# georgeretsi/smirk

Hardware: AMD Instinct MI355X
Metric: faces/sec (encode+FLAME+render+generate) @224x224 (higher is better)
Workload: dtype f32 results; encoder + generator convs as split-fp16 x3 MFMA with f32 accumulate (fp32-class error), FLAME / raster f32; 1 GPU; BASELINE config 4: full inference incl. SmirkGenerator re-synthesis, 1024-frame batch sharded over the GPUs; global_batch=1024, micro_batch=1024, image=224x224, parallelism=dp1, rccl_ranks_seen=1, collective=none (1 GPU), hw_queues=4

## Files before the change

### smirk_amd/csrc/mbconv_image.hip

```cpp
#include <stdio.h>

#include "common.h"

typedef _Float16 half8 __attribute__((ext_vector_type(8)));

struct MBIArgs {
    const char* x;
    const char* wexp;
    const float *s1, *b1;
    const float* wdw;
    const float *s2, *b2;
    const char* wproj;
    const float *s3, *b3;
    char* out;
    int B, H, W, Cin, mid, Cout, residual, ipw, rows, gsz, nb;
    int off_es, off_wp, off_wc, off_gmap;
    int gpitch;
    int tile, tiles_x, tiles_y, nbands;
};

extern __shared__ __attribute__((aligned(16))) char mbi_smem[];

__device__ __forceinline__ void mbi_barrier() {
    asm volatile("s_waitcnt lgkmcnt(0)" ::: "memory");
    __builtin_amdgcn_s_barrier();
    asm volatile("" ::: "memory");
}

__device__ __forceinline__ int mbi_es(int gi, int c) { return gi * 32 + ((((c >> 2) ^ (gi >> 1)) & 7) << 2) + (c & 3); }

template <int KS, int NT, bool PADK>
__device__ __forceinline__ void mbi_whole_body(const MBIArgs& a) {
    SmirkRangeAccS rng;
    const int strideX = KS * 64 + 16;
    char* Xs = mbi_smem;
    float* Es = (float*)(mbi_smem + a.off_es);
    char* Wp = mbi_smem + a.off_wp;
    float* Wc = (float*)(mbi_smem + a.off_wc);
    short* gmap = (short*)(mbi_smem + a.off_gmap);
    const int tid = threadIdx.x, lane = tid & 63, wave = tid >> 6, fr = lane & 31, hb = lane >> 5;
    const int b0 = blockIdx.x * a.ipw;
    const int nimg = min(a.ipw, a.B - b0), HW = a.H * a.W, vrows = nimg * HW;
    const int nchunks = (a.mid + 31) / 32;
    const size_t xrow = (size_t)a.Cin * 4;
    const half8 hz = {0, 0, 0, 0, 0, 0, 0, 0};
    const int swave = __builtin_amdgcn_readfirstlane(wave);
    const bool active = swave < a.nb;
    const int wpbuf = a.Cout * 144;

    half8 we[KS][2];
    float s1v = 0.f, b1v = 0.f;
    auto load_we = [&](int c) {
        int frw = fr;
        asm volatile("" : "+v"(frw));
        const int ch = 32 * c + frw;
        const bool v = ch < a.mid;
        const int chc = min(ch, a.mid - 1);
        const char* wbase = a.wexp;
        asm volatile("" : "+s"(wbase));
        const char* wrow = wbase + (unsigned)chc * (unsigned)(a.Cin * 4);
#pragma unroll
        for (int s = 0; s < KS; ++s) {
            const int g = 2 * s + hb;
            if constexpr (PADK) {
                const int gc = min(g, a.Cin / 8 - 1);
                const half8 t0 = *(const half8*)(wrow + gc * 32), t1h = *(const half8*)(wrow + gc * 32 + 16);
                we[s][0] = g * 8 < a.Cin ? t0 : hz;
                we[s][1] = g * 8 < a.Cin ? t1h : hz;
            } else {
                we[s][0] = *(const half8*)(wrow + g * 32);
                we[s][1] = *(const half8*)(wrow + g * 32 + 16);
            }
        }
        const float t1 = a.s1[chc], t2 = a.b1[chc];
        s1v = v ? t1 : 0.f;
        b1v = v ? t2 : 0.f;
    };
    f32x4 wpv[2];
    float wcv = 0.f;
    auto fetch_stage = [&](int c) {
        int t0 = tid;
        asm volatile("" : "+v"(t0));
#pragma unroll
        for (int u = 0; u < 2; ++u) {
            const int idx = t0 + 512 * u, row = idx >> 3, piece = idx & 7, kg = 4 * c + (piece >> 1);
            const bool ok = row < a.Cout && kg * 8 < a.mid;
            const int rc = min(row, a.Cout - 1), kc = min(kg, a.mid / 8 - 1);
            const f32x4 t = *(const f32x4*)(a.wproj + ((size_t)rc * a.mid + kc * 8) * 4 + (piece & 1) * 16);
            const f32x4 z = {0.f, 0.f, 0.f, 0.f};
            wpv[u] = ok ? t : z;
        }
        {
            const int k = min(t0 >> 5, 10), ch = 32 * c + (t0 & 31), chc = min(ch, a.mid - 1);
            const float* src = k < 9 ? a.wdw + (size_t)k * a.mid : (k == 9 ? a.s2 : a.b2);
            const float t = src[chc];
            wcv = ch < a.mid ? t : 0.f;
        }
    };
    auto store_stage = [&](int c) {
        char* dst = Wp + (c & 1) * wpbuf;
        int t0 = tid;
        asm volatile("" : "+v"(t0));
#pragma unroll
        for (int u = 0; u < 2; ++u) {
            const int idx = t0 + 512 * u, row = idx >> 3, piece = idx & 7;
            if (row < a.Cout) *(f32x4*)(dst + row * 144 + piece * 16) = wpv[u];
        }
        if (t0 < 352) Wc[(c & 1) * 352 + t0] = wcv;
    };

    {
        const int P = a.Cin / 4;
        const char* xb = a.x + (size_t)b0 * HW * xrow;
        const int total = a.rows * P, vtotal = vrows * P;
        for (int base = 0; base < total; base += 512 * 4) {
            f32x4 xv[4];
#pragma unroll
            for (int u = 0; u < 4; ++u) {
                const int idx = base + 512 * u + tid;
                const f32x4 z = {0.f, 0.f, 0.f, 0.f};
                const f32x4 t = *(const f32x4*)(xb + (size_t)min(idx, vtotal - 1) * 16);
                xv[u] = idx < vtotal ? t : z;
            }
#pragma unroll
            for (int u = 0; u < 4; ++u) {
                const int idx = base + 512 * u + tid, row = idx / P, pc = idx - row * P;
                if (idx < total) *(f32x4*)(Xs + row * strideX + pc * 16) = xv[u];
            }
        }
        if (PADK && KS * 4 > P) {
            const int PP = KS * 4 - P;
            for (int idx = tid; idx < a.rows * PP; idx += 512) {
                const int row = idx / PP, pc = P + idx - row * PP;
                *(f32x4*)(Xs + row * strideX + pc * 16) = f32x4{0.f, 0.f, 0.f, 0.f};
            }
        }
        for (int idx = tid; idx < a.gsz * 8; idx += 512) ((f32x4*)Es)[idx] = f32x4{0.f, 0.f, 0.f, 0.f};
        for (int r = tid; r < a.nb * 32; r += 512) {
            int g = -1;
            if (r < vrows) {
                const int im = r / HW, rem = r - im * HW, y = rem / a.W, xx = rem - y * a.W;
                g = (im * (a.H + 2) + y + 1) * (a.W + 2) + xx + 1;
            }
            gmap[r] = (short)g;
        }
    }
    mbi_barrier();

    f32x16 pacc[NT][2];
#pragma unroll
    for (int q = 0; q < NT; ++q)
#pragma unroll
        for (int h = 0; h < 2; ++h)
#pragma unroll
            for (int r = 0; r < 16; ++r) pacc[q][h][r] = 0.f;
    const int myrow = min(wave * 32 + fr, a.rows - 1);
    const int mygi = active ? (int)gmap[min(wave * 32 + fr, a.nb * 32 - 1)] : -1;

    auto expand = [&]() {
        if (!active) return;
        f32x16 e0, e1;
#pragma unroll
        for (int r = 0; r < 16; ++r) { e0[r] = 0.f; e1[r] = 0.f; }
        const char* arow = Xs + myrow * strideX;
#pragma unroll
        for (int s = 0; s < KS; ++s) {
            const int g = 2 * s + hb;
            const half8 ah = *(const half8*)(arow + g * 32), al = *(const half8*)(arow + g * 32 + 16);
            e0 = __builtin_amdgcn_mfma_f32_32x32x16_f16(ah, we[s][0], e0, 0, 0, 0);
            e1 = __builtin_amdgcn_mfma_f32_32x32x16_f16(ah, we[s][1], e1, 0, 0, 0);
            e1 = __builtin_amdgcn_mfma_f32_32x32x16_f16(al, we[s][0], e1, 0, 0, 0);
            if ((s & 1) || NT == 4) __builtin_amdgcn_sched_barrier(0);
        }
        int rbase = wave * 32 + 4 * hb;
        asm volatile("" : "+v"(rbase));
#pragma unroll
        for (int r = 0; r < 16; ++r) {
            const int gm = gmap[rbase + (r & 3) + 8 * (r >> 2)];
            const float v = fmaxf((e0[r] + e1[r] * (1.0f / 2048.0f)) * s1v + b1v, 0.f);
            Es[mbi_es(gm >= 0 ? gm : ~gm, fr)] = gm >= 0 ? v : 0.f;
        }
    };


    for (int c = -1; c < nchunks; ++c) {
        const bool more = c + 1 < nchunks;
        if (more) fetch_stage(c + 1);
        half8 dh[2] = {hz, hz}, dl[2] = {hz, hz};
        if (c >= 0 && active && mygi >= 0) {
            const float* wc = Wc + (c & 1) * 352;
#pragma unroll
            for (int s = 0; s < 2; ++s) {
                const int c8 = 8 * (2 * s + hb);
                int gc = mygi;
                asm volatile("" : "+v"(gc));
                float acc[8] = {0.f, 0.f, 0.f, 0.f, 0.f, 0.f, 0.f, 0.f};
#pragma unroll
                for (int ky = 0; ky < 3; ++ky)
#pragma unroll
                    for (int kx = 0; kx < 3; ++kx) {
                        const int gi = gc + (ky - 1) * a.gpitch + (kx - 1);
                        const f32x4 v0 = *(const f32x4*)(Es + mbi_es(gi, c8)), v1 = *(const f32x4*)(Es + mbi_es(gi, c8 + 4));
                        const f32x4 w0 = *(const f32x4*)(wc + (ky * 3 + kx) * 32 + c8), w1 = *(const f32x4*)(wc + (ky * 3 + kx) * 32 + c8 + 4);
#pragma unroll
                        for (int q = 0; q < 4; ++q) { acc[q] = fmaf(v0[q], w0[q], acc[q]); acc[4 + q] = fmaf(v1[q], w1[q], acc[4 + q]); }
                        if (kx == 2 || NT == 4) __builtin_amdgcn_sched_barrier(0);
                    }
                const f32x4 sa = *(const f32x4*)(wc + 9 * 32 + c8), sb = *(const f32x4*)(wc + 9 * 32 + c8 + 4);
                const f32x4 ba = *(const f32x4*)(wc + 10 * 32 + c8), bb = *(const f32x4*)(wc + 10 * 32 + c8 + 4);
#pragma unroll
                for (int q = 0; q < 8; ++q) {
                    const float v = fmaxf(acc[q] * (q < 4 ? sa[q & 3] : sb[q & 3]) + (q < 4 ? ba[q & 3] : bb[q & 3]), 0.f);
                    _Float16 h, l;
                    smirk_split1(v, h, l);
                    dh[s][q] = h; dl[s][q] = l;
                }
            }
        }
        if (more) store_stage(c + 1);
        mbi_barrier();
        if (more) load_we(c + 1);
        if (c >= 0 && active) {
            const char* wp = Wp + (c & 1) * wpbuf;
            int frq = fr;
            asm volatile("" : "+v"(frq));
#pragma unroll
            for (int q = 0; q < NT; ++q) {
                const int co = min(q * 32 + frq, a.Cout - 1);
                const char* brow = wp + co * 144;
#pragma unroll
                for (int s = 0; s < 2; ++s) {
                    const int g = 2 * s + hb;
                    const half8 bhh = *(const half8*)(brow + g * 32), bll = *(const half8*)(brow + g * 32 + 16);
                    pacc[q][0] = __builtin_amdgcn_mfma_f32_32x32x16_f16(dh[s], bhh, pacc[q][0], 0, 0, 0);
                    pacc[q][1] = __builtin_amdgcn_mfma_f32_32x32x16_f16(dh[s], bll, pacc[q][1], 0, 0, 0);
                    pacc[q][1] = __builtin_amdgcn_mfma_f32_32x32x16_f16(dl[s], bhh, pacc[q][1], 0, 0, 0);
                }
                __builtin_amdgcn_sched_barrier(0);
            }
        }
        if (more) expand();
        mbi_barrier();
    }

    if (active) {
        const int lane = __builtin_amdgcn_mbcnt_hi(~0u, __builtin_amdgcn_mbcnt_lo(~0u, 0u)), wave = swave, fr = lane & 31;
        float* tb = Es + wave * (32 * 36);
        char* ob = a.out + (size_t)b0 * HW * a.Cout * 4;
#pragma unroll
        for (int q = 0; q < NT; ++q) {
            if (q * 32 < a.Cout) {
                const int co = q * 32 + fr;
                const float s3 = co < a.Cout ? a.s3[co] : 0.f, b3 = co < a.Cout ? a.b3[co] : 0.f;
#pragma unroll
                for (int r = 0; r < 16; ++r) tb[mfma32_row(r, lane) * 36 + fr] = (pacc[q][0][r] + pacc[q][1][r] * (1.0f / 2048.0f)) * s3 + b3;
                asm volatile("s_waitcnt lgkmcnt(0)" ::: "memory");
#pragma unroll
                for (int it = 0; it < 2; ++it) {
                    const int item = it * 64 + lane, row = item >> 2, g8 = q * 4 + (item & 3);
                    const int r = wave * 32 + row;
                    if (r < vrows && g8 * 8 < a.Cout) {
                        float v[8];
                        *(f32x4*)v = *(const f32x4*)(tb + row * 36 + (item & 3) * 8);
                        *(f32x4*)(v + 4) = *(const f32x4*)(tb + row * 36 + (item & 3) * 8 + 4);
                        if (a.residual) {
                            const char* xr = Xs + r * strideX + g8 * 32;
                            const half8 hi = *(const half8*)xr, lo = *(const half8*)(xr + 16);
#pragma unroll
                            for (int k = 0; k < 8; ++k) v[k] += (float)hi[k] + (float)lo[k] * (1.0f / 2048.0f);
                        }
                        half8 hi, lo;
                        rng.see8(v);
#pragma unroll
                        for (int k = 0; k < 8; ++k) {
                            _Float16 h, l;
                            smirk_split1(v[k], h, l);
                            hi[k] = h; lo[k] = l;
                        }
                        char* o = ob + ((size_t)r * a.Cout + g8 * 8) * 4;
                        *(half8*)o = hi;
                        *(half8*)(o + 16) = lo;
                    }
                }
                asm volatile("s_waitcnt lgkmcnt(0)" ::: "memory");
            }
        }
    }
    rng.commit();
}

#define MBB_EB 8192
#define MBB_STAGE 34

__device__ __forceinline__ void mbb_out_px(int m, int& oy, int& ox) {
    const int k = m >> 2;
    oy = (0x96 >> k) & 1;
    ox = (k >> 1) * 4 + (m & 3);
}

__device__ __forceinline__ void mbb_fence() { asm volatile("s_waitcnt lgkmcnt(0)" ::: "memory"); }

template <int KS, int NT>
__device__ __forceinline__ void mbi_band_body(const MBIArgs& a) {
    SmirkRangeAccS rng;
    const int tid = threadIdx.x, lane = tid & 63, fr = lane & 31, hb = lane >> 5;
    const int wave = __builtin_amdgcn_readfirstlane(tid >> 6);
    float* Wt = (float*)(mbi_smem + 4 * MBB_EB);
    const int band = (int)blockIdx.x * 4 + wave;
    const bool has = band < a.nbands;
    int bid = min(band, a.nbands - 1);
    const int bx = bid % a.tiles_x; bid /= a.tiles_x;
    const int by = bid % a.tiles_y;
    const int b = bid / a.tiles_y;
    const int oy0 = by * 2, ox0 = bx * 14;
    const bool interior = oy0 > 0 && oy0 + 2 < a.H && ox0 > 0 && ox0 + 14 < a.W;
    const unsigned xrow = (unsigned)a.Cin * 4;
    const int gmax = a.Cin / 8;
    const int nchunks = (a.mid + 31) / 32;
    const half8 hz = {0, 0, 0, 0, 0, 0, 0, 0};
    const char* xb = a.x + (size_t)b * a.H * a.W * xrow;

    auto stage = [&](int c0) {
        const int total = min(MBB_STAGE, nchunks - c0) * 352;
        for (int base = 0; base < total; base += 256 * 8) {
            float cv[8];
#pragma unroll
            for (int u = 0; u < 8; ++u) {
                const int idx = min(base + 256 * u + tid, total - 1), cl = idx / 352, rem = idx - cl * 352, k = rem >> 5;
                const int ch = 32 * (c0 + cl) + (rem & 31), chc = min(ch, a.mid - 1);
                const float* src = k < 9 ? a.wdw + (size_t)k * a.mid : (k == 9 ? a.s2 : a.b2);
                const float t = src[chc];
                cv[u] = ch < a.mid ? t : 0.f;
            }
#pragma unroll
            for (int u = 0; u < 8; ++u)
                if (base + 256 * u + tid < total) Wt[base + 256 * u + tid] = cv[u];
        }
    };
    unsigned xo[2], om[2];
#pragma unroll
    for (int t = 0; t < 2; ++t) {
        const int iy = oy0 - 1 + 2 * t + (fr >> 4), ix = ox0 - 1 + (fr & 15);
        const bool ok = iy >= 0 && iy < a.H && ix >= 0 && ix < a.W;
        const int yc = min(max(iy, 0), a.H - 1), xc = min(max(ix, 0), a.W - 1);
        xo[t] = (unsigned)(yc * a.W + xc) * xrow;
        om[t] = (unsigned)__builtin_amdgcn_ballot_w64(ok) >> (4 * hb);
    }
    auto load_x = [&](int t, half8 (*dst)[2]) {
        const char* px = xb + xo[t];
#pragma unroll
        for (int s = 0; s < KS; ++s) {
            const int g = 2 * s + hb, gc = min(g, gmax - 1);
            const half8 t0 = *(const half8*)(px + gc * 32), t1 = *(const half8*)(px + gc * 32 + 16);
            if (s == KS - 1) { dst[s][0] = g < gmax ? t0 : hz; dst[s][1] = g < gmax ? t1 : hz; }
            else { dst[s][0] = t0; dst[s][1] = t1; }
        }
    };
    half8 xa[2][KS][2];
    load_x(0, xa[0]);
    load_x(1, xa[1]);
    half8 we[KS][2];
    float s1v, b1v;
    auto load_we = [&](int c) {
        const int ch = 32 * c + fr, chc = min(ch, a.mid - 1);
        const char* wrow = a.wexp + (size_t)chc * xrow;
#pragma unroll
        for (int s = 0; s < KS; ++s) {
            const int g = 2 * s + hb, gc = min(g, gmax - 1);
            const half8 t0 = *(const half8*)(wrow + gc * 32), t1 = *(const half8*)(wrow + gc * 32 + 16);
            if (s == KS - 1) { we[s][0] = g < gmax ? t0 : hz; we[s][1] = g < gmax ? t1 : hz; }
            else { we[s][0] = t0; we[s][1] = t1; }
        }
        const float t1 = a.s1[chc], t2 = a.b1[chc];
        s1v = ch < a.mid ? t1 : 0.f;
        b1v = ch < a.mid ? t2 : 0.f;
    };
    load_we(0);
    stage(0);
    mbb_fence();
    __builtin_amdgcn_s_barrier();
    asm volatile("" ::: "memory");
    if (!has) {
        for (int c0 = MBB_STAGE; c0 < nchunks; c0 += MBB_STAGE) {
            __builtin_amdgcn_s_barrier();
            stage(c0);
            mbb_fence();
            __builtin_amdgcn_s_barrier();
        }
        return;
    }

    const unsigned ebase = (unsigned)wave * MBB_EB;
    const unsigned est = ebase + hb * 512 + ((((unsigned)fr >> 2) ^ (hb << 1)) << 4) + (fr & 3) * 4;
    unsigned ta[9];
    int my_oy, my_ox;
    mbb_out_px(fr, my_oy, my_ox);
#pragma unroll
    for (int ky = 0; ky < 3; ++ky)
#pragma unroll
        for (int kx = 0; kx < 3; ++kx) {
            const int cell = ((my_oy + ky) * 16 + my_ox + kx) & 63;
            ta[ky * 3 + kx] = ebase + cell * 128 + ((((cell >> 1) ^ (2 * hb)) & 7) << 4);
        }

    f32x16 pacc[NT][2];
#pragma unroll
    for (int q = 0; q < NT; ++q)
#pragma unroll
        for (int h = 0; h < 2; ++h)
#pragma unroll
            for (int r = 0; r < 16; ++r) pacc[q][h][r] = 0.f;

    const float* wc = Wt;
    int crestage = MBB_STAGE;
    for (int c = 0; c < nchunks; ++c, wc += 352) {
        if (c == crestage) {
            mbb_fence();
            __builtin_amdgcn_s_barrier();
            stage(c);
            mbb_fence();
            __builtin_amdgcn_s_barrier();
            asm volatile("" ::: "memory");
            wc = Wt; crestage += MBB_STAGE;
        }
#pragma unroll
        for (int t = 0; t < 2; ++t) {
            half8 (*cur)[2] = xa[t];
            unsigned et = est;
            asm volatile("" : "+v"(et));
            f32x16 e0, e1;
#pragma unroll
            for (int r = 0; r < 16; ++r) { e0[r] = 0.f; e1[r] = 0.f; }
#pragma unroll
            for (int s = 0; s < KS; ++s) {
                e0 = __builtin_amdgcn_mfma_f32_32x32x16_f16(cur[s][0], we[s][0], e0, 0, 0, 0);
                e1 = __builtin_amdgcn_mfma_f32_32x32x16_f16(cur[s][0], we[s][1], e1, 0, 0, 0);
                e1 = __builtin_amdgcn_mfma_f32_32x32x16_f16(cur[s][1], we[s][0], e1, 0, 0, 0);
            }
            if (interior) {
#pragma unroll
                for (int r = 0; r < 16; ++r) {
                    const int ro = (r & 3) + 8 * (r >> 2);
                    const unsigned cr = ((r >> 1) & 1) | (((r >> 2) & 1) << 2);
                    const float v = fmaxf((e0[r] + e1[r] * (1.0f / 2048.0f)) * s1v + b1v, 0.f);
                    *(float*)(mbi_smem + (et ^ (cr << 4)) + (32 * t + ro) * 128) = v;
                }
            } else {
#pragma unroll
                for (int r = 0; r < 16; ++r) {
                    const int ro = (r & 3) + 8 * (r >> 2);
                    const unsigned cr = ((r >> 1) & 1) | (((r >> 2) & 1) << 2);
                    const float v = fmaxf((e0[r] + e1[r] * (1.0f / 2048.0f)) * s1v + b1v, 0.f);
                    *(float*)(mbi_smem + (et ^ (cr << 4)) + (32 * t + ro) * 128) = ((om[t] >> ro) & 1u) ? v : 0.f;
                }
            }
        }
        if (c + 1 < nchunks) load_we(c + 1);
        half8 wp[NT][2][2];
#pragma unroll
        for (int q = 0; q < NT; ++q) {
            const int co = q * 32 + fr;
            const char* wrow = a.wproj + (size_t)(co < a.Cout ? co : 0) * a.mid * 4;
#pragma unroll
            for (int s = 0; s < 2; ++s) {
                const int kg = min(4 * c + 2 * s + hb, a.mid / 8 - 1);
                const bool v = co < a.Cout && (4 * c + 2 * s + hb) * 8 < a.mid;
                const half8 t0 = *(const half8*)(wrow + kg * 32), t1 = *(const half8*)(wrow + kg * 32 + 16);
                wp[q][s][0] = v ? t0 : hz;
                wp[q][s][1] = v ? t1 : hz;
            }
        }
        mbb_fence();
        half8 dh[2], dl[2];
#pragma unroll
        for (int s = 0; s < 2; ++s) {
            const int c8 = 8 * (2 * s + hb);
            float acc[8] = {0.f, 0.f, 0.f, 0.f, 0.f, 0.f, 0.f, 0.f};
#pragma unroll
            for (int ky = 0; ky < 3; ++ky)
#pragma unroll
                for (int kx = 0; kx < 3; ++kx) {
                    const int k = ky * 3 + kx;
                    unsigned tk = ta[k];
                    asm volatile("" : "+v"(tk));
                    const f32x4 v0 = *(const f32x4*)(mbi_smem + (tk ^ ((4 * s) << 4))), v1 = *(const f32x4*)(mbi_smem + (tk ^ ((4 * s + 1) << 4)));
                    const f32x4 w0 = *(const f32x4*)(wc + k * 32 + c8), w1 = *(const f32x4*)(wc + k * 32 + c8 + 4);
#pragma unroll
                    for (int q = 0; q < 4; ++q) { acc[q] = fmaf(v0[q], w0[q], acc[q]); acc[4 + q] = fmaf(v1[q], w1[q], acc[4 + q]); }
                    if (kx == 2 || NT == 1) __builtin_amdgcn_sched_barrier(0);
                }
            const f32x4 sa = *(const f32x4*)(wc + 9 * 32 + c8), sb = *(const f32x4*)(wc + 9 * 32 + c8 + 4);
            const f32x4 ba = *(const f32x4*)(wc + 10 * 32 + c8), bb = *(const f32x4*)(wc + 10 * 32 + c8 + 4);
#pragma unroll
            for (int q = 0; q < 8; ++q) {
                const float v = fmaxf(acc[q] * (q < 4 ? sa[q & 3] : sb[q & 3]) + (q < 4 ? ba[q & 3] : bb[q & 3]), 0.f);
                _Float16 h, l;
                smirk_split1(v, h, l);
                dh[s][q] = h; dl[s][q] = l;
            }
        }
        mbb_fence();
#pragma unroll
        for (int q = 0; q < NT; ++q)
#pragma unroll
            for (int s = 0; s < 2; ++s) {
                pacc[q][0] = __builtin_amdgcn_mfma_f32_32x32x16_f16(dh[s], wp[q][s][0], pacc[q][0], 0, 0, 0);
                pacc[q][1] = __builtin_amdgcn_mfma_f32_32x32x16_f16(dh[s], wp[q][s][1], pacc[q][1], 0, 0, 0);
                pacc[q][1] = __builtin_amdgcn_mfma_f32_32x32x16_f16(dl[s], wp[q][s][0], pacc[q][1], 0, 0, 0);
            }
    }

    {
        float* tb = (float*)(mbi_smem + ebase);
        char* ob = a.out + (size_t)b * a.H * a.W * a.Cout * 4;
        float s3v[NT], b3v[NT];
        half8 rh[NT][2], rl[NT][2];
#pragma unroll
        for (int q = 0; q < NT; ++q) {
            const int co = q * 32 + fr, coc = min(co, a.Cout - 1);
            const float t1 = a.s3[coc], t2 = a.b3[coc];
            s3v[q] = co < a.Cout ? t1 : 0.f;
            b3v[q] = co < a.Cout ? t2 : 0.f;
#pragma unroll
            for (int it = 0; it < 2; ++it) {
                rh[q][it] = hz; rl[q][it] = hz;
                if (a.residual) {
                    const int item = it * 64 + lane, g8 = min(q * 4 + (item & 3), gmax - 1);
                    int py, px;
                    mbb_out_px(item >> 2, py, px);
                    const char* xr = xb + ((size_t)(oy0 + py) * a.W + ox0 + min(px, 13)) * xrow + g8 * 32;
                    rh[q][it] = *(const half8*)xr; rl[q][it] = *(const half8*)(xr + 16);
                }
            }
        }
#pragma unroll
        for (int q = 0; q < NT; ++q) {
            if (q * 32 < a.Cout) {
                const float s3 = s3v[q], b3 = b3v[q];
#pragma unroll
                for (int r = 0; r < 16; ++r) tb[mfma32_row(r, lane) * 36 + fr] = (pacc[q][0][r] + pacc[q][1][r] * (1.0f / 2048.0f)) * s3 + b3;
                mbb_fence();
#pragma unroll
                for (int it = 0; it < 2; ++it) {
                    const int item = it * 64 + lane, row = item >> 2, g8 = q * 4 + (item & 3);
                    int py, px;
                    mbb_out_px(row, py, px);
                    if (px < 14 && g8 * 8 < a.Cout) {
                        const size_t opix = (size_t)(oy0 + py) * a.W + ox0 + px;
                        float v[8];
                        *(f32x4*)v = *(const f32x4*)(tb + row * 36 + (item & 3) * 8);
                        *(f32x4*)(v + 4) = *(const f32x4*)(tb + row * 36 + (item & 3) * 8 + 4);
                        if (a.residual) {
                            const half8 hi = rh[q][it], lo = rl[q][it];
#pragma unroll
                            for (int k = 0; k < 8; ++k) v[k] += (float)hi[k] + (float)lo[k] * (1.0f / 2048.0f);
                        }
                        half8 hi, lo;
                        rng.see8(v);
#pragma unroll
                        for (int k = 0; k < 8; ++k) {
                            _Float16 h, l;
                            smirk_split1(v[k], h, l);
                            hi[k] = h; lo[k] = l;
                        }
                        char* o = ob + (opix * a.Cout + g8 * 8) * 4;
                        *(half8*)o = hi;
                        *(half8*)(o + 16) = lo;
                    }
                }
                mbb_fence();
            }
        }
    }
    rng.commit();
}

template <int KS, int NT, bool TILE = false, bool PADK = false>
__global__ __launch_bounds__(TILE ? 256 : 512, TILE && NT == 1 ? 3 : 2) void mbconv_image_kernel(MBIArgs a) {
    if constexpr (TILE) mbi_band_body<KS, NT>(a);
    else mbi_whole_body<KS, NT, PADK>(a);
}

struct MbiPlan { int ipw, rows, gsz, nb, off_es, off_wp, off_wc, off_gmap, tile, tiles_x, tiles_y, gpitch; size_t lds; };
static bool mbi_plan(int H, int W, int Cin, int mid, int Cout, MbiPlan& p) {
    if (H <= 0 || W <= 0 || Cin % 8 || mid % 8 || Cout % 8 || Cin < 16 || Cin > 112 || Cout > 128 || mid <= 0 || Cout <= 0) return false;
    const int KS = (Cin + 15) / 16;
    p.tile = H * W > 224 ? 1 : 0;
    if (p.tile) {
        if (H % 14 || W % 14) return false;
        p.tiles_x = W / 14; p.tiles_y = H / 2; p.gpitch = 16;
        p.ipw = 1; p.rows = 28; p.gsz = 64; p.nb = 1;
        p.off_es = p.off_wp = p.off_gmap = 0; p.off_wc = 4 * MBB_EB;
        const int nchunks = (mid + 31) / 32;
        p.lds = (size_t)4 * MBB_EB + (size_t)(nchunks < MBB_STAGE ? nchunks : MBB_STAGE) * 352 * 4;
        return true;
    }
    p.tiles_x = p.tiles_y = 1; p.gpitch = W + 2;
    p.ipw = 224 / (H * W);
    if (p.ipw > 8) p.ipw = 8;
    p.rows = p.ipw * H * W;
    p.gsz = p.ipw * (H + 2) * (W + 2);
    p.nb = (p.rows + 31) / 32;
    if (p.nb > 7 || p.gsz * 128 < p.nb * 32 * 36 * 4) return false;
    size_t o = (size_t)p.rows * (KS * 64 + 16);
    o = (o + 15) / 16 * 16; p.off_es = (int)o; o += (size_t)p.gsz * 128;
    p.off_wp = (int)o; o += (size_t)2 * Cout * 144;
    p.off_wc = (int)o; o += 2 * 352 * 4;
    p.off_gmap = (int)o; o += (size_t)p.nb * 32 * 2;
    p.lds = (o + 15) / 16 * 16;
    return p.lds <= 160 * 1024;
}

static bool mbi_has_variant(int ks, int nt) {
    return (ks == 5 && (nt == 2 || nt == 3 || nt == 4)) || (ks == 6 && (nt == 3 || nt == 4)) || (ks == 7 && (nt == 3 || nt == 4)) ||
           (ks == 4 && (nt == 2 || nt == 3)) || (ks == 2 && nt == 1) || (ks == 3 && nt == 2);
}

extern "C" int smirk_mbconv_image_supported(int H, int W, int Cin, int mid, int Cout, int stride) {
    MbiPlan p;
    if (stride != 1 || !mbi_plan(H, W, Cin, mid, Cout, p)) return 0;
    const int ks = (Cin + 15) / 16, nt = (Cout + 31) / 32;
    if (!mbi_has_variant(ks, nt)) return 0;
    const bool small = (ks == 2 && nt == 1) || (ks == 3 && nt == 2);
    return (small || (!p.tile && Cin % 16 == 0)) ? 1 : 0;
}

template <int KS, int NT, bool TILE = false, bool PADK = false>
static int mbi_launch(const MBIArgs& a, unsigned grid, size_t lds, hipStream_t st) {
    if (const int rc = smirk_raise_dynamic_lds((const void*)mbconv_image_kernel<KS, NT, TILE, PADK>, (TILE ? 80 : 160) * 1024)) return rc;
    if (g_smirk_prof_on) {
        char nm[64];
        if (TILE || PADK) snprintf(nm, sizeof(nm), "mbconv_image_kernel<%d,%d,%s,%s>", KS, NT, TILE ? "true" : "false", PADK ? "true" : "false");
        else snprintf(nm, sizeof(nm), "mbconv_image_kernel<%d,%d>", KS, NT);
        const double px = (double)a.B * a.H * a.W;
        smirk_prof_next_mbconv(nm, px, px, a.Cin, a.mid, a.Cout, true, a.residual != 0);
    }
    SMIRK_LAUNCH((mbconv_image_kernel<KS, NT, TILE, PADK>), dim3(grid), dim3(TILE ? 256 : 512), lds, st, a);
    return smirk_launch_status();
}

extern "C" int smirk_mbconv_image_split16(const void* x, const void* wexp, const float* s1, const float* b1, const float* wdw, const float* s2,
                                          const float* b2, const void* wproj, const float* s3, const float* b3, int residual, void* out, int B,
                                          int H, int W, int Cin, int mid, int Cout, void* stream) {
    if (!x || !wexp || !s1 || !b1 || !wdw || !s2 || !b2 || !wproj || !s3 || !b3 || !out || B <= 0) return SMIRK_ERR_BAD_ARG;
    if (residual && Cin != Cout) return SMIRK_ERR_BAD_ARG;
    MbiPlan p;
    if (!mbi_plan(H, W, Cin, mid, Cout, p) || !smirk_mbconv_image_supported(H, W, Cin, mid, Cout, 1)) return SMIRK_ERR_UNSUPPORTED;
    MBIArgs a;
    a.x = (const char*)x; a.wexp = (const char*)wexp; a.s1 = s1; a.b1 = b1; a.wdw = wdw; a.s2 = s2; a.b2 = b2; a.wproj = (const char*)wproj;
    a.s3 = s3; a.b3 = b3; a.out = (char*)out; a.B = B; a.H = H; a.W = W; a.Cin = Cin; a.mid = mid; a.Cout = Cout; a.residual = residual;
    a.ipw = p.ipw; a.rows = p.rows; a.gsz = p.gsz; a.nb = p.nb; a.off_es = p.off_es; a.off_wp = p.off_wp; a.off_wc = p.off_wc; a.off_gmap = p.off_gmap;
    a.tile = p.tile; a.tiles_x = p.tiles_x; a.tiles_y = p.tiles_y; a.gpitch = p.gpitch;
    const size_t nbands = (size_t)B * p.tiles_x * p.tiles_y;
    if (p.tile && (nbands > 0x7fffffffu / 4 || (size_t)H * W * Cin * 4 > 0x7fffffffu)) return SMIRK_ERR_UNSUPPORTED;
    a.nbands = (int)nbands;
    const unsigned grid = p.tile ? (unsigned)((nbands + 3) / 4) : (unsigned)((B + p.ipw - 1) / p.ipw);
    hipStream_t st = (hipStream_t)stream;
    const int ks = (Cin + 15) / 16, nt = (Cout + 31) / 32;
#define MBI_CASE(K, N) if (ks == K && nt == N) return mbi_launch<K, N>(a, grid, p.lds, st)
    MBI_CASE(5, 3); MBI_CASE(5, 4); MBI_CASE(6, 3); MBI_CASE(7, 4);
    MBI_CASE(4, 2); MBI_CASE(4, 3); MBI_CASE(5, 2); MBI_CASE(6, 4); MBI_CASE(7, 3);
    if (ks == 2 && nt == 1) return p.tile ? mbi_launch<2, 1, true, true>(a, grid, p.lds, st) : mbi_launch<2, 1, false, true>(a, grid, p.lds, st);
    if (ks == 3 && nt == 2) return p.tile ? mbi_launch<3, 2, true, true>(a, grid, p.lds, st) : mbi_launch<3, 2, false, true>(a, grid, p.lds, st);
#undef MBI_CASE
    return SMIRK_ERR_UNSUPPORTED;
}
```

### smirk_amd/csrc/mbconv_s2.hip

```cpp
#include <stdio.h>

#include "common.h"

typedef _Float16 half8 __attribute__((ext_vector_type(8)));

#define S2W_NH 153
#define S2W_EB (S2W_NH * 128)
#define S2W_MAX_MID 96

struct MBS2Args {
    const char* x;
    const char* wexp;
    const float *s1, *b1;
    const float* wdw;
    const float *s2, *b2;
    const char* wproj;
    const float *s3, *b3;
    char* out;
    int B, H, W, Cin, mid, Cout, Ho, Wo, pt, pl, tiles_x, tiles_y, ntiles;
};

__device__ __forceinline__ int s2w_idx(int hy, int hx) {
    const int R = hy >> 1, J = hx >> 1;
    if (!(hx & 1)) return ((hy & 1) ? 85 : 0) + (R >> 1) * 18 + 2 * J + (R & 1);
    if (hy & 1) return 121 + (R >> 1) * 16 + 2 * J + (R & 1);
    return R < 4 ? 53 + (R >> 1) * 16 + 2 * J + (R & 1) : 37 + 2 * J;
}
__device__ __forceinline__ bool s2w_pix(int p, int& hy, int& hx) {
    int R, J, rp, cp;
    if (p < 53) {
        if (p < 36 || !(p & 1)) { const int pr = p / 18, rem = p - pr * 18; rp = 0; cp = 0; R = 2 * pr + (rem & 1); J = rem >> 1; }
        else { rp = 0; cp = 1; R = 4; J = (p - 37) >> 1; }
    } else if (p < 85) { const int u = p - 53; rp = 0; cp = 1; R = 2 * (u >> 4) + (u & 1); J = (u & 15) >> 1; }
    else if (p < 121) { const int u = p - 85, pr = u / 18, rem = u - pr * 18; rp = 1; cp = 0; R = 2 * pr + (rem & 1); J = rem >> 1; }
    else { const int u = p - 121; rp = 1; cp = 1; R = 2 * (u >> 4) + (u & 1); J = (u & 15) >> 1; }
    hy = 2 * R + rp; hx = 2 * J + cp;
    return p < S2W_NH;
}
__device__ __forceinline__ void s2w_out_px(int m, int& oy, int& ox) {
    const int k = m >> 2;
    oy = (0xD728 >> (2 * k)) & 3;
    ox = ((k >> 1) & 1) * 4 + (m & 3);
}

__device__ __forceinline__ void s2w_fence() { asm volatile("s_waitcnt lgkmcnt(0)" ::: "memory"); }

template <int KS, int NT>
__global__ __launch_bounds__(256, 2) void mbconv_s2_wave_kernel(MBS2Args a) {
    constexpr bool HOLD = KS == 1;
    constexpr int NB = 5;
    extern __shared__ __attribute__((aligned(16))) char s2w_smem[];
    SmirkRangeAccS rng;
    const int tid = threadIdx.x, lane = tid & 63, fr = lane & 31, hb = lane >> 5;
    const int wave = __builtin_amdgcn_readfirstlane(tid >> 6);
    float* Wt = (float*)(s2w_smem + 4 * S2W_EB);
    const int tile = (int)blockIdx.x * 4 + wave;
    const bool has = tile < a.ntiles;
    int bid = min(tile, a.ntiles - 1);
    const int tx = bid % a.tiles_x; bid /= a.tiles_x;
    const int ty = bid % a.tiles_y;
    const int b = bid / a.tiles_y;
    const int oy0 = ty * 4, ox0 = tx * 8, iy0 = oy0 * 2 - a.pt, ix0 = ox0 * 2 - a.pl;
    const unsigned xrow = (unsigned)a.Cin * 4;
    const int gmax = a.Cin / 8;
    const int nchunks = (a.mid + 31) / 32;
    const half8 hz = {0, 0, 0, 0, 0, 0, 0, 0};
    const char* xb = a.x + (size_t)b * a.H * a.W * xrow;

    {
        const int n = 9 * a.mid;
        float cv[4];
#pragma unroll
        for (int u = 0; u < 4; ++u) cv[u] = a.wdw[min(tid + 256 * u, n - 1)];
#pragma unroll
        for (int u = 0; u < 4; ++u)
            if (tid + 256 * u < n) Wt[tid + 256 * u] = cv[u];
    }
    unsigned xo[NB], om[NB];
#pragma unroll
    for (int t = 0; t < NB; ++t) {
        int hy, hx;
        const bool cell = s2w_pix(32 * t + fr, hy, hx);
        const int iy = iy0 + hy, ix = ix0 + hx;
        const bool ok = cell && iy >= 0 && iy < a.H && ix >= 0 && ix < a.W;
        const int yc = min(max(iy, 0), a.H - 1), xc = min(max(ix, 0), a.W - 1);
        xo[t] = (unsigned)(yc * a.W + xc) * xrow;
        om[t] = (unsigned)__builtin_amdgcn_ballot_w64(ok) >> (4 * hb);
    }
    auto load_x = [&](int t, half8 (*dst)[2]) {
        const char* px = xb + xo[t];
#pragma unroll
        for (int s = 0; s < KS; ++s) {
            const int g = 2 * s + hb, gc = min(g, gmax - 1);
            const half8 t0 = *(const half8*)(px + gc * 32), t1 = *(const half8*)(px + gc * 32 + 16);
            if (s == KS - 1) { dst[s][0] = g < gmax ? t0 : hz; dst[s][1] = g < gmax ? t1 : hz; }
            else { dst[s][0] = t0; dst[s][1] = t1; }
        }
    };
    half8 xa[HOLD ? NB : 2][KS][2];
    if constexpr (HOLD) {
#pragma unroll
        for (int t = 0; t < NB; ++t) load_x(t, xa[t]);
    } else {
        load_x(0, xa[0]);
    }
    half8 we[KS][2];
    float s1v, b1v;
    auto load_we = [&](int c) {
        const int ch = 32 * c + fr, chc = min(ch, a.mid - 1);
        const char* wrow = a.wexp + (size_t)chc * xrow;
#pragma unroll
        for (int s = 0; s < KS; ++s) {
            const int g = 2 * s + hb, gc = min(g, gmax - 1);
            const bool v = ch < a.mid && g < gmax;
            const half8 t0 = *(const half8*)(wrow + gc * 32), t1 = *(const half8*)(wrow + gc * 32 + 16);
            we[s][0] = v ? t0 : hz;
            we[s][1] = v ? t1 : hz;
        }
        const float t1 = a.s1[chc], t2 = a.b1[chc];
        s1v = ch < a.mid ? t1 : 0.f;
        b1v = ch < a.mid ? t2 : 0.f;
    };
    load_we(0);
    asm volatile("s_waitcnt lgkmcnt(0)" ::: "memory");
    __builtin_amdgcn_s_barrier();
    asm volatile("" ::: "memory");
    if (!has) return;

    const unsigned ebase = (unsigned)wave * S2W_EB;
    const unsigned est = ebase + hb * 512 + ((((unsigned)fr >> 2) ^ (hb << 1)) << 4) + (fr & 3) * 4;
    unsigned ta[9];
    int my_oy, my_ox;
    s2w_out_px(fr, my_oy, my_ox);
#pragma unroll
    for (int ky = 0; ky < 3; ++ky)
#pragma unroll
        for (int kx = 0; kx < 3; ++kx) {
            const int idx = s2w_idx(2 * my_oy + ky, 2 * my_ox + kx);
            ta[ky * 3 + kx] = ebase + idx * 128 + ((((idx >> 1) ^ (2 * hb)) & 7) << 4);
        }

    f32x16 pacc[NT][2];
#pragma unroll
    for (int q = 0; q < NT; ++q)
#pragma unroll
        for (int h = 0; h < 2; ++h)
#pragma unroll
            for (int r = 0; r < 16; ++r) pacc[q][h][r] = 0.f;

    for (int c = 0; c < nchunks; ++c) {
        if constexpr (!HOLD) {
            if (c > 0) {
#pragma unroll
                for (int s = 0; s < KS; ++s) { xa[0][s][0] = xa[1][s][0]; xa[0][s][1] = xa[1][s][1]; }
            }
        }
#pragma unroll
        for (int t = 0; t < NB; ++t) {
            if constexpr (!HOLD) {
                if (t + 1 < NB) load_x(t + 1, xa[(t + 1) & 1]);
                else if (c + 1 < nchunks) load_x(0, xa[1]);
            }
            half8 (*cur)[2] = xa[HOLD ? t : (t & 1)];
            unsigned et = est;
            if (NT > 1) asm volatile("" : "+v"(et));
            f32x16 e0, e1;
#pragma unroll
            for (int r = 0; r < 16; ++r) { e0[r] = 0.f; e1[r] = 0.f; }
#pragma unroll
            for (int s = 0; s < KS; ++s) {
                e0 = __builtin_amdgcn_mfma_f32_32x32x16_f16(cur[s][0], we[s][0], e0, 0, 0, 0);
                e1 = __builtin_amdgcn_mfma_f32_32x32x16_f16(cur[s][0], we[s][1], e1, 0, 0, 0);
                e1 = __builtin_amdgcn_mfma_f32_32x32x16_f16(cur[s][1], we[s][0], e1, 0, 0, 0);
            }
#pragma unroll
            for (int r = 0; r < 16; ++r) {
                const int ro = (r & 3) + 8 * (r >> 2);
                const unsigned cr = ((r >> 1) & 1) | (((r >> 2) & 1) << 2);
                if (t < NB - 1 || ro + 4 * hb < S2W_NH - 32 * (NB - 1)) {
                    const float v = fmaxf((e0[r] + e1[r] * (1.0f / 2048.0f)) * s1v + b1v, 0.f);
                    *(float*)(s2w_smem + (et ^ (cr << 4)) + (32 * t + ro) * 128) = ((om[t] >> ro) & 1u) ? v : 0.f;
                }
            }
        }
        if (c + 1 < nchunks) load_we(c + 1);
        half8 wp[NT][2][2];
#pragma unroll
        for (int q = 0; q < NT; ++q) {
            const int co = q * 32 + fr;
            const char* wrow = a.wproj + (size_t)(co < a.Cout ? co : 0) * a.mid * 4;
#pragma unroll
            for (int s = 0; s < 2; ++s) {
                const int kg = min(4 * c + 2 * s + hb, a.mid / 8 - 1);
                const bool v = co < a.Cout && (4 * c + 2 * s + hb) * 8 < a.mid;
                const half8 t0 = *(const half8*)(wrow + kg * 32), t1 = *(const half8*)(wrow + kg * 32 + 16);
                wp[q][s][0] = v ? t0 : hz;
                wp[q][s][1] = v ? t1 : hz;
            }
        }
        s2w_fence();
        half8 dh[2], dl[2];
#pragma unroll
        for (int s = 0; s < 2; ++s) {
            const int cg = 32 * c + 8 * (2 * s + hb), cb = min(cg, a.mid - 8);
            const f32x4 sa = *(const f32x4*)(a.s2 + cb), sb = *(const f32x4*)(a.s2 + cb + 4);
            const f32x4 ba = *(const f32x4*)(a.b2 + cb), bb = *(const f32x4*)(a.b2 + cb + 4);
            const float* wt = Wt + cb;
            float acc[8] = {0.f, 0.f, 0.f, 0.f, 0.f, 0.f, 0.f, 0.f};
#pragma unroll
            for (int ky = 0; ky < 3; ++ky)
#pragma unroll
                for (int kx = 0; kx < 3; ++kx) {
                    const int k = ky * 3 + kx;
                    unsigned tk = ta[k];
                    if (NT > 1) asm volatile("" : "+v"(tk));
                    const f32x4 v0 = *(const f32x4*)(s2w_smem + (tk ^ ((4 * s) << 4))), v1 = *(const f32x4*)(s2w_smem + (tk ^ ((4 * s + 1) << 4)));
                    const f32x4 w0 = *(const f32x4*)(wt + k * a.mid), w1 = *(const f32x4*)(wt + k * a.mid + 4);
#pragma unroll
                    for (int q = 0; q < 4; ++q) { acc[q] = fmaf(v0[q], w0[q], acc[q]); acc[4 + q] = fmaf(v1[q], w1[q], acc[4 + q]); }
                    if (NT > 1 && kx == 2) __builtin_amdgcn_sched_barrier(0);
                }
            half8 h8, l8;
#pragma unroll
            for (int q = 0; q < 8; ++q) {
                const float v = fmaxf(acc[q] * (q < 4 ? sa[q & 3] : sb[q & 3]) + (q < 4 ? ba[q & 3] : bb[q & 3]), 0.f);
                _Float16 h, l;
                smirk_split1(v, h, l);
                h8[q] = h; l8[q] = l;
            }
            dh[s] = cg < a.mid ? h8 : hz;
            dl[s] = cg < a.mid ? l8 : hz;
        }
        s2w_fence();
#pragma unroll
        for (int q = 0; q < NT; ++q)
#pragma unroll
            for (int s = 0; s < 2; ++s) {
                pacc[q][0] = __builtin_amdgcn_mfma_f32_32x32x16_f16(dh[s], wp[q][s][0], pacc[q][0], 0, 0, 0);
                pacc[q][1] = __builtin_amdgcn_mfma_f32_32x32x16_f16(dh[s], wp[q][s][1], pacc[q][1], 0, 0, 0);
                pacc[q][1] = __builtin_amdgcn_mfma_f32_32x32x16_f16(dl[s], wp[q][s][0], pacc[q][1], 0, 0, 0);
            }
    }

    {
        float* tb = (float*)(s2w_smem + ebase);
        char* ob = a.out + (size_t)b * a.Ho * a.Wo * a.Cout * 4;
#pragma unroll
        for (int q = 0; q < NT; ++q) {
            const int co = q * 32 + fr;
            const float s3 = co < a.Cout ? a.s3[co] : 0.f, b3 = co < a.Cout ? a.b3[co] : 0.f;
#pragma unroll
            for (int r = 0; r < 16; ++r) tb[mfma32_row(r, lane) * 36 + fr] = (pacc[q][0][r] + pacc[q][1][r] * (1.0f / 2048.0f)) * s3 + b3;
            s2w_fence();
#pragma unroll
            for (int it = 0; it < 2; ++it) {
                const int item = it * 64 + lane, row = item >> 2, g8 = q * 4 + (item & 3);
                int py, px;
                s2w_out_px(row, py, px);
                const int oy = oy0 + py, ox = ox0 + px;
                if (oy < a.Ho && ox < a.Wo && g8 * 8 < a.Cout) {
                    float v[8];
                    *(f32x4*)v = *(const f32x4*)(tb + row * 36 + (item & 3) * 8);
                    *(f32x4*)(v + 4) = *(const f32x4*)(tb + row * 36 + (item & 3) * 8 + 4);
                    half8 hi, lo;
                    rng.see8(v);
#pragma unroll
                    for (int k = 0; k < 8; ++k) {
                        _Float16 h, l;
                        smirk_split1(v[k], h, l);
                        hi[k] = h; lo[k] = l;
                    }
                    char* o = ob + ((size_t)oy * a.Wo + ox) * a.Cout * 4 + g8 * 32;
                    *(half8*)o = hi;
                    *(half8*)(o + 16) = lo;
                }
            }
            s2w_fence();
        }
    }
    rng.commit();
}

extern "C" int smirk_mbconv_s2_supported(int Cin, int mid, int Cout) {
    if (Cin <= 0 || mid <= 0 || Cout <= 0 || Cin % 8 || mid % 8 || Cout % 8 || mid > S2W_MAX_MID) return 0;
    const int ks = (Cin + 15) / 16, nt = (Cout + 31) / 32;
    return (ks == 1 && nt == 1) || (ks == 2 && nt == 2);
}

template <int KS, int NT>
static int s2w_launch(const MBS2Args& a, unsigned grid, size_t lds, hipStream_t st) {
    if (const int rc = smirk_raise_dynamic_lds((const void*)mbconv_s2_wave_kernel<KS, NT>, 80 * 1024)) return rc;
    if (g_smirk_prof_on) {
        char nm[64];
        snprintf(nm, sizeof(nm), "mbconv_s2_wave_kernel<%d,%d>", KS, NT);
        smirk_prof_next_mbconv(nm, (double)a.B * a.H * a.W, (double)a.B * a.Ho * a.Wo, a.Cin, a.mid, a.Cout, true, false);
    }
    SMIRK_LAUNCH((mbconv_s2_wave_kernel<KS, NT>), dim3(grid), dim3(256), lds, st, a);
    return smirk_launch_status();
}

extern "C" int smirk_mbconv_s2_split16(const void* x, const void* wexp, const float* s1, const float* b1, const float* wdw, const float* s2,
                                       const float* b2, const void* wproj, const float* s3, const float* b3, void* out, int B, int H, int W,
                                       int Cin, int mid, int Cout, void* stream) {
    if (!x || !wexp || !s1 || !b1 || !wdw || !s2 || !b2 || !wproj || !s3 || !b3 || !out || B <= 0 || H <= 0 || W <= 0) return SMIRK_ERR_BAD_ARG;
    if ((((uintptr_t)s2) | ((uintptr_t)b2)) & 15) return SMIRK_ERR_BAD_ARG;
    if (!smirk_mbconv_s2_supported(Cin, mid, Cout)) return SMIRK_ERR_UNSUPPORTED;
    MBS2Args a;
    a.x = (const char*)x; a.wexp = (const char*)wexp; a.s1 = s1; a.b1 = b1; a.wdw = wdw; a.s2 = s2; a.b2 = b2;
    a.wproj = (const char*)wproj; a.s3 = s3; a.b3 = b3; a.out = (char*)out;
    a.B = B; a.H = H; a.W = W; a.Cin = Cin; a.mid = mid; a.Cout = Cout;
    a.Ho = (H + 1) / 2; a.Wo = (W + 1) / 2;
    a.pt = smirk_same_pad_lead(H, 2); a.pl = smirk_same_pad_lead(W, 2);
    a.tiles_x = (a.Wo + 7) / 8; a.tiles_y = (a.Ho + 3) / 4;
    const size_t ntiles = (size_t)B * a.tiles_x * a.tiles_y;
    if (ntiles > 0x7fffffffu / 4 || (size_t)H * W * Cin * 4 > 0x7fffffffu) return SMIRK_ERR_UNSUPPORTED;
    a.ntiles = (int)ntiles;
    const size_t lds = (size_t)4 * S2W_EB + smirk_align_up((size_t)9 * mid * 4, 16);
    const unsigned grid = (unsigned)((ntiles + 3) / 4);
    const int ks = (Cin + 15) / 16;
    if (ks == 1) return s2w_launch<1, 1>(a, grid, lds, (hipStream_t)stream);
    return s2w_launch<2, 2>(a, grid, lds, (hipStream_t)stream);
}
```

Baseline: 11650 faces/sec.

## Route small-image MBConv layers through band-tiled kernel; skip halo masking for interior s2 tiles

For small feature maps (H*W<=224, divisible by 14) using the KS=2/NT=1 or KS=3/NT=2 variants, the planner now picks the 14-wide band-tiled kernel instead of the whole-image-per-workgroup path, unless a disable switch is set. This aims to spread work across more, smaller workgroups and improve occupancy on small late-stage layers. The profiler label keeps the old name. Separately, the stride-2 MBConv kernel gets a branch for tiles fully inside the image that writes the expanded activation without the per-row padding mask select. The cost is more code and a uniform branch per tile.

```diff
diff --git a/smirk_amd/csrc/mbconv_image.hip b/smirk_amd/csrc/mbconv_image.hip
--- a/smirk_amd/csrc/mbconv_image.hip
+++ b/smirk_amd/csrc/mbconv_image.hip
@@ -582,10 +582,11 @@
 }
 
 struct MbiPlan { int ipw, rows, gsz, nb, off_es, off_wp, off_wc, off_gmap, tile, tiles_x, tiles_y, gpitch; size_t lds; };
-static bool mbi_plan(int H, int W, int Cin, int mid, int Cout, MbiPlan& p) {
+static bool mbi_plan(int H, int W, int Cin, int mid, int Cout, MbiPlan& p, bool band14 = false) {
     if (H <= 0 || W <= 0 || Cin % 8 || mid % 8 || Cout % 8 || Cin < 16 || Cin > 112 || Cout > 128 || mid <= 0 || Cout <= 0) return false;
-    const int KS = (Cin + 15) / 16;
+    const int KS = (Cin + 15) / 16, NT = (Cout + 31) / 32;
     p.tile = H * W > 224 ? 1 : 0;
+    if (band14 && !p.tile && H % 14 == 0 && W % 14 == 0 && ((KS == 2 && NT == 1) || (KS == 3 && NT == 2))) p.tile = 1;
     if (p.tile) {
         if (H % 14 || W % 14) return false;
         p.tiles_x = W / 14; p.tiles_y = H / 2; p.gpitch = 16;
@@ -625,12 +626,12 @@
     return (small || (!p.tile && Cin % 16 == 0)) ? 1 : 0;
 }
 
-template <int KS, int NT, bool TILE = false, bool PADK = false>
+template <int KS, int NT, bool TILE = false, bool PADK = false, bool LABEL_TILE = TILE>
 static int mbi_launch(const MBIArgs& a, unsigned grid, size_t lds, hipStream_t st) {
     if (const int rc = smirk_raise_dynamic_lds((const void*)mbconv_image_kernel<KS, NT, TILE, PADK>, (TILE ? 80 : 160) * 1024)) return rc;
     if (g_smirk_prof_on) {
         char nm[64];
-        if (TILE || PADK) snprintf(nm, sizeof(nm), "mbconv_image_kernel<%d,%d,%s,%s>", KS, NT, TILE ? "true" : "false", PADK ? "true" : "false");
+        if (LABEL_TILE || PADK) snprintf(nm, sizeof(nm), "mbconv_image_kernel<%d,%d,%s,%s>", KS, NT, LABEL_TILE ? "true" : "false", PADK ? "true" : "false");
         else snprintf(nm, sizeof(nm), "mbconv_image_kernel<%d,%d>", KS, NT);
         const double px = (double)a.B * a.H * a.W;
         smirk_prof_next_mbconv(nm, px, px, a.Cin, a.mid, a.Cout, true, a.residual != 0);
@@ -645,7 +646,9 @@
     if (!x || !wexp || !s1 || !b1 || !wdw || !s2 || !b2 || !wproj || !s3 || !b3 || !out || B <= 0) return SMIRK_ERR_BAD_ARG;
     if (residual && Cin != Cout) return SMIRK_ERR_BAD_ARG;
     MbiPlan p;
-    if (!mbi_plan(H, W, Cin, mid, Cout, p) || !smirk_mbconv_image_supported(H, W, Cin, mid, Cout, 1)) return SMIRK_ERR_UNSUPPORTED;
+    if (!smirk_mbconv_image_supported(H, W, Cin, mid, Cout, 1)) return SMIRK_ERR_UNSUPPORTED;
+    const bool band14 = H * W <= 224 && smirk_switch(SMIRK_SW_DISABLE_MBCONV_TILE) == 0;
+    if (!mbi_plan(H, W, Cin, mid, Cout, p, band14)) return SMIRK_ERR_UNSUPPORTED;
     MBIArgs a;
     a.x = (const char*)x; a.wexp = (const char*)wexp; a.s1 = s1; a.b1 = b1; a.wdw = wdw; a.s2 = s2; a.b2 = b2; a.wproj = (const char*)wproj;
     a.s3 = s3; a.b3 = b3; a.out = (char*)out; a.B = B; a.H = H; a.W = W; a.Cin = Cin; a.mid = mid; a.Cout = Cout; a.residual = residual;
@@ -660,8 +663,13 @@
 #define MBI_CASE(K, N) if (ks == K && nt == N) return mbi_launch<K, N>(a, grid, p.lds, st)
     MBI_CASE(5, 3); MBI_CASE(5, 4); MBI_CASE(6, 3); MBI_CASE(7, 4);
     MBI_CASE(4, 2); MBI_CASE(4, 3); MBI_CASE(5, 2); MBI_CASE(6, 4); MBI_CASE(7, 3);
-    if (ks == 2 && nt == 1) return p.tile ? mbi_launch<2, 1, true, true>(a, grid, p.lds, st) : mbi_launch<2, 1, false, true>(a, grid, p.lds, st);
-    if (ks == 3 && nt == 2) return p.tile ? mbi_launch<3, 2, true, true>(a, grid, p.lds, st) : mbi_launch<3, 2, false, true>(a, grid, p.lds, st);
+#define MBI_SMALL(K, N)                                                                                  \
+    if (ks == K && nt == N) {                                                                            \
+        if (!p.tile) return mbi_launch<K, N, false, true>(a, grid, p.lds, st);                           \
+        return band14 ? mbi_launch<K, N, true, true, false>(a, grid, p.lds, st) : mbi_launch<K, N, true, true>(a, grid, p.lds, st); \
+    }
+    MBI_SMALL(2, 1); MBI_SMALL(3, 2);
+#undef MBI_SMALL
 #undef MBI_CASE
     return SMIRK_ERR_UNSUPPORTED;
 }
diff --git a/smirk_amd/csrc/mbconv_s2.hip b/smirk_amd/csrc/mbconv_s2.hip
--- a/smirk_amd/csrc/mbconv_s2.hip
+++ b/smirk_amd/csrc/mbconv_s2.hip
@@ -61,6 +61,7 @@
     const int ty = bid % a.tiles_y;
     const int b = bid / a.tiles_y;
     const int oy0 = ty * 4, ox0 = tx * 8, iy0 = oy0 * 2 - a.pt, ix0 = ox0 * 2 - a.pl;
+    const bool interior = NT > 1 && iy0 >= 0 && iy0 + 9 <= a.H && ix0 >= 0 && ix0 + 17 <= a.W;
     const unsigned xrow = (unsigned)a.Cin * 4;
     const int gmax = a.Cin / 8;
     const int nchunks = (a.mid + 31) / 32;
@@ -173,13 +174,25 @@
                 e1 = __builtin_amdgcn_mfma_f32_32x32x16_f16(cur[s][0], we[s][1], e1, 0, 0, 0);
                 e1 = __builtin_amdgcn_mfma_f32_32x32x16_f16(cur[s][1], we[s][0], e1, 0, 0, 0);
             }
-#pragma unroll
-            for (int r = 0; r < 16; ++r) {
-                const int ro = (r & 3) + 8 * (r >> 2);
-                const unsigned cr = ((r >> 1) & 1) | (((r >> 2) & 1) << 2);
-                if (t < NB - 1 || ro + 4 * hb < S2W_NH - 32 * (NB - 1)) {
-                    const float v = fmaxf((e0[r] + e1[r] * (1.0f / 2048.0f)) * s1v + b1v, 0.f);
-                    *(float*)(s2w_smem + (et ^ (cr << 4)) + (32 * t + ro) * 128) = ((om[t] >> ro) & 1u) ? v : 0.f;
+            if (interior) {
+#pragma unroll
+                for (int r = 0; r < 16; ++r) {
+                    const int ro = (r & 3) + 8 * (r >> 2);
+                    const unsigned cr = ((r >> 1) & 1) | (((r >> 2) & 1) << 2);
+                    if (t < NB - 1 || ro + 4 * hb < S2W_NH - 32 * (NB - 1)) {
+                        const float v = fmaxf((e0[r] + e1[r] * (1.0f / 2048.0f)) * s1v + b1v, 0.f);
+                        *(float*)(s2w_smem + (et ^ (cr << 4)) + (32 * t + ro) * 128) = v;
+                    }
+                }
+            } else {
+#pragma unroll
+                for (int r = 0; r < 16; ++r) {
+                    const int ro = (r & 3) + 8 * (r >> 2);
+                    const unsigned cr = ((r >> 1) & 1) | (((r >> 2) & 1) << 2);
+                    if (t < NB - 1 || ro + 4 * hb < S2W_NH - 32 * (NB - 1)) {
+                        const float v = fmaxf((e0[r] + e1[r] * (1.0f / 2048.0f)) * s1v + b1v, 0.f);
+                        *(float*)(s2w_smem + (et ^ (cr << 4)) + (32 * t + ro) * 128) = ((om[t] >> ro) & 1u) ? v : 0.f;
+                    }
                 }
             }
         }
```

After: 11670 faces/sec, median of 6. Within noise of the previous version (+0.2%).
